# achinastone/Tensorium

Hardware: AMD Instinct MI355X
Metric: fp32 SGEMM GFLOP/s (M=N=K=4096) + YOLOv3 conv-fwd images/s (higher is better)
Workload: dtype fp32; 1 GPU; sgemm_nn_4096x4096x4096; M=4096, N=4096, K=4096, parallelism=1 independent replicas, one process per GPU, no data-path collective

## Files before the change

include/tns.h:

```cpp
#ifndef TNS_H
#define TNS_H

#include <stdint.h>
#include <stddef.h>

#ifdef __cplusplus
extern "C" {
#endif

#define TNS_ABI_VERSION 1

enum { TNS_CblasRowMajor = 101, TNS_CblasColMajor = 102 };
enum { TNS_CblasNoTrans = 111, TNS_CblasTrans = 112 };

enum {
  TNS_acLOGISTIC = 0, TNS_acRELU = 1, TNS_acRELU6 = 2, TNS_acRELIE = 3,
  TNS_acLINEAR = 4, TNS_acRAMP = 5, TNS_acTANH = 6, TNS_acPLSE = 7,
  TNS_acREVLEAKY = 8, TNS_acLEAKY = 9, TNS_acELU = 10, TNS_acLOGGY = 11,
  TNS_acSTAIR = 12, TNS_acHARDTAN = 13, TNS_acLHTAN = 14, TNS_acSELU = 15
};

enum {
  TNS_OK = 0,
  TNS_ERR_ARG = 1,
// ... 321 lines not shown
int         tns_conv_dw_tile_count(void);
int         tns_conv_tile_variant_count(void);
const char* tns_conv_tile_variant_name(int32_t variant);
int         tns_conv_slab_count(void);
const char* tns_conv_slab_name(int32_t variant);
int         tns_conv1x1_count(void);
const char* tns_conv1x1_name(int32_t variant);
int         tns_sdot_chains_variant_count(void);
const char* tns_sdot_chains_variant_name(int32_t variant);
int         tns_sdot_rc_variant_count(void);
const char* tns_sdot_rc_variant_name(int32_t variant);
const char* tns_gemm_variant_name(int32_t variant);
int tns_hip_gemm_variant(tns_ctx* ctx, int32_t variant, uint8_t transA, uint8_t transB,
                         int64_t M, int64_t N, int64_t K, float ALPHA,
                         const float* A, int64_t aOffset, int64_t lda, int64_t strideA,
                         const float* B, int64_t bOffset, int64_t ldb, int64_t strideB,
                         float BETA, float* C, int64_t cOffset, int64_t ldc, int64_t strideC,
                         int64_t batchCount);

enum { TNS_OPT_STRICT_BETA0 = 0, TNS_OPT_CONV_VARIANT = 1, TNS_OPT_CONV_PAD = 2,
       TNS_OPT_NT_SDOT = 3, TNS_OPT_SRSS_QUIRK = 4, TNS_OPT_TT_EXACT = 5,
       TNS_OPT_SDOT_FORM = 6, TNS_OPT_DX_FUSED = 7, TNS_OPT_DX_TILE = 8,
       TNS_OPT_DW_TILE = 9, TNS_OPT_BWD_OVERLAP = 10, TNS_OPT_DX_CONV = 11,
       TNS_OPT_DW_RES = 12, TNS_OPT_DERIVE_SUMS = 13, TNS_OPT_SCRATCH_CAP = 14 };
int tns_set_option(int32_t opt, int64_t value);

#ifdef __cplusplus
}
#endif
#endif
```

tensorium_amd/_abi.py:

```python
from __future__ import annotations

import ctypes as C
import os
import re
from pathlib import Path

PKG = Path(__file__).resolve().parent
ROOT = PKG.parent
LIB_PATH = PKG / "libtensorium_hip.so"
HEADER = ROOT / "include" / "tns.h"

i32, i64, u8, f32 = C.c_int32, C.c_int64, C.c_uint8, C.c_float
fptr = C.c_void_p
vp = C.c_void_p

CblasRowMajor, CblasColMajor = 101, 102
CblasNoTrans, CblasTrans = 111, 112
ACT = dict(LOGISTIC=0, RELU=1, RELU6=2, RELIE=3, LINEAR=4, RAMP=5, TANH=6, PLSE=7,
           REVLEAKY=8, LEAKY=9, ELU=10, LOGGY=11, STAIR=12, HARDTAN=13, LHTAN=14, SELU=15)
TNS_OK = 0
TNS_OP_GEMM, TNS_OP_IM2COL, TNS_OP_COL2IM, TNS_OP_BIAS, TNS_OP_ACTIVATE = range(5)
TNS_OPT_STRICT_BETA0 = 0
TNS_OPT_CONV_VARIANT, TNS_OPT_CONV_PAD, TNS_OPT_NT_SDOT, TNS_OPT_SRSS_QUIRK = 1, 2, 3, 4
TNS_OPT_TT_EXACT = 5
TNS_OPT_SDOT_FORM = 6
TNS_OPT_DX_FUSED = 7
TNS_OPT_DX_TILE = 8
TNS_OPT_DW_TILE = 9
TNS_OPT_BWD_OVERLAP = 10
TNS_OPT_DX_CONV = 11
TNS_OPT_DW_RES = 12
TNS_OPT_DERIVE_SUMS = 13
TNS_OPT_SCRATCH_CAP = 14

_CONV = [i64] * 11

PROTOTYPES: dict[str, tuple] = {
    "tns_abi_version": (C.c_int, []),
    "tns_last_error": (C.c_char_p, []),
    "tns_clear_error": (None, []),
    "tns_set_error_hook": (None, [vp]),
    "tns_device_count": (C.c_int, []),
    "tns_set_option": (C.c_int, [i32, i64]),
    "tns_cblas_sgemm": (None, [i32, i32, i32, i64, i64, i64, f32, fptr, i64, fptr, i64, f32,
                               fptr, i64]),
    "tns_cblas_sgemm_batch_strided": (None, [i32, i32, i32, i64, i64, i64, f32, fptr, i64, i64,
                                             fptr, i64, i64, f32, fptr, i64, i64, i64]),
    "tns_im2col": (None, [*_CONV, fptr, i64, fptr, i64, u8]),
    "tns_col2im": (None, [*_CONV, fptr, i64, fptr, i64, i64, u8]),
    "tns_im2col_strided_batched": (None, [*_CONV, fptr, i64, i64, fptr, i64, i64, i64]),
    "tns_col2im_strided_batched": (None, [*_CONV, fptr, i64, i64, fptr, i64, i64, i64]),
    "tns_hip_create": (C.c_int, [i32, C.POINTER(vp)]),
    "tns_hip_destroy": (C.c_int, [vp]),
    "tns_hip_set_stream": (C.c_int, [vp, vp]),
    "tns_hip_get_stream": (vp, [vp]),
    "tns_hip_pending_dw": (C.c_int, [vp]),
# ... 174 lines not shown
```

tensorium_amd/csrc/sgemm_nn_big.hip:

```cpp
#include <type_traits>

#include "tns_internal.hpp"

namespace tns {
namespace {

typedef float floatx16 __attribute__((ext_vector_type(16)));

template <int BM, int BN, int WM, int WN, int MINB, int BK = 32>
struct Geo {
  static constexpr int BM_ = BM, BN_ = BN, WN_ = WN, MINB_ = MINB, BK_ = BK;
  static constexpr int KQ = BK / 4;
  static constexpr int NT = 64 * WM * WN;
  static constexpr int WTM = BM / WM, WTN = BN / WN;
  static constexpr int TM = WTM / 32, TN = WTN / 32;
  static constexpr int LDA = BM, LDB = BN;
  static constexpr int A_TILE = BK * LDA, B_TILE = BK * LDB;
  static constexpr int STAGE = A_TILE + B_TILE;
  static constexpr int AU = BM * BK / 4 / NT;
  static constexpr int BROWS = 256 / BN;
  static constexpr int BDMA = BK / BROWS / (NT / 64);
  static_assert(TM == 2 || TM == 4, "A fragments read as one b64 / b128");
  static_assert(BN == 128 || BN == 256, "B rows of 512 B or 1 KB per DMA");
  static_assert(AU >= 1 && BDMA >= 1 && BM * BK / 4 % NT == 0, "staging split");
// ... 220 lines not shown
}

template <class G>
hipError_t launch(const GemmArgs& a, hipStream_t s) {
  if (!applies<G>(a)) return hipErrorInvalidValue;
  const int64_t tiles = (a.M / G::BM_) * (a.N / G::BN_);
  for (int64_t b0 = 0; b0 < a.batch; b0 += 65535) {
    GemmArgs sub = a;
    const int64_t nb = a.batch - b0 < 65535 ? a.batch - b0 : 65535;
    sub.A = a.A + b0 * a.strideA;
    sub.B = a.B + b0 * a.strideB;
    sub.C = a.C + b0 * a.strideC;
    sub.batch = nb;
    hipLaunchKernelGGL(sgemm_nn_big_kernel<G>, dim3((unsigned)tiles, (unsigned)nb), dim3(G::NT), 0,
                       s, sub);
    hipError_t e = hipGetLastError();
    if (e != hipSuccess) return e;
  }
  return hipSuccess;
}

}

int sgemm_nn_big_count() { return 9; }
const char* sgemm_nn_big_name(int v) {
  static const char* names[] = {"256x256x32_w2x4_nn_big", "128x128x32_w2x2_nn_big",
                                "256x128x32_w2x2_nn_big", "256x256x32_w4x4_nn_big",
                                "256x128x16_w2x2_b2_nn_big", "256x256x32_w2x4_pp_nn_big",
                                "256x256x32_w2x2_dma_nn_big", "256x256x32_w2x2_dma_flat_nn_big",
                                "256x256x32_w2x2_dma_b32_nn_big"};
  return v >= 0 && v < sgemm_nn_big_count() ? names[v] : "";
}

int sgemm_nn_big_pick(const GemmArgs& a) {
  if (applies<G256>(a) && (a.M / 256) * (a.N / 256) * a.batch >= 192)
    return sgemm_nn_w4_applies(a) ? 6 : sgemm_nn_pp_applies(a) ? 5 : 0;
  return -1;
}

hipError_t launch_sgemm_nn_big(int v, const GemmArgs& a, hipStream_t s) {
  switch (v) {
    case 0: return launch<G256>(a, s);
    case 1: return launch<G128>(a, s);
    case 2: return launch<G256x128>(a, s);
    case 3: return launch<G256w16>(a, s);
    case 4: return launch<G256x128k16>(a, s);
    case 5: return launch_sgemm_nn_pp(a, s);
    case 6: return launch_sgemm_nn_w4(a, s, true);
    case 7: return launch_sgemm_nn_w4(a, s, false);
    case 8: return launch_sgemm_nn_w4(a, s, true, false);
    default: return hipErrorInvalidValue;
  }
}

}
```

tensorium_amd/csrc/sgemm_nn_w4.hip:

```cpp
#include <type_traits>

#include "tns_internal.hpp"

namespace tns {
namespace {

typedef float floatx16 __attribute__((ext_vector_type(16)));
typedef float floatx4 __attribute__((ext_vector_type(4)));
typedef int int4v __attribute__((ext_vector_type(4)));
typedef const __attribute__((address_space(3))) float* lds_cptr;
typedef const __attribute__((address_space(3))) floatx4* lds_cptr4;

constexpr int BM = 256, BN = 256, BK = 32, NT = 256;
constexpr int A_TILE = BM * BK, B_TILE = BK * BN, STAGE = A_TILE + B_TILE;
constexpr int ROWS_MIN_TILES = 4;
constexpr int PRE_MIN_TILES = 8;

__device__ __forceinline__ void dma16(const float* sbase, unsigned voff, unsigned lds) {
  unsigned keep;
  asm volatile(
      "s_mov_b32 %0, m0\n\ts_mov_b32 m0, %3\n\ts_nop 0\n\t"
      "global_load_lds_dwordx4 %1, %2\n\ts_mov_b32 m0, %0"
      : "=&s"(keep)
      : "v"(voff), "s"(sbase), "s"(lds)
      : "memory");
}

#ifdef TNS_W4_STAMPS
#define TNS_W4_STAMP(i) stamp[i] = __builtin_amdgcn_s_memtime()
#else
#define TNS_W4_STAMP(i) \
  do {                  \
  } while (0)
#endif

template <bool ALPHA1, bool ROWS, bool PRE>
__global__ __launch_bounds__(NT, 1) void sgemm_nn_w4_kernel(GemmArgs p) {
  __shared__ __attribute__((aligned(16))) float smem[2 * STAGE];
#ifdef TNS_W4_STAMPS
  unsigned long long stamp[4];
  TNS_W4_STAMP(0);
#endif
  const int tid = threadIdx.x, lane = tid & 63;
  const int wid = __builtin_amdgcn_readfirstlane(tid >> 6);
  const int lc = lane & 31, h = lane >> 5;
  const int wm = wid >> 1, wn = wid & 1;

  const int tiles_m = (int)(p.M / BM), tiles_n = (int)(p.N / BN);
  int tm, tn;
  const int64_t bz = blockIdx.y;
  {
    const int nb = tiles_m * tiles_n, bid = blockIdx.x;
    const int xcd = bid & 7, q = nb >> 3, r = nb & 7;
    const int wg = (xcd < r ? xcd * (q + 1) : r * (q + 1) + (xcd - r) * q) + (bid >> 3);
    constexpr int GROUP_M = 8;
    const int per_group = GROUP_M * tiles_n;
    const int group = wg / per_group, first_m = group * GROUP_M;
    const int gsize = min(tiles_m - first_m, GROUP_M);
    const int in_group = wg - group * per_group;
    tm = first_m + in_group % gsize;
    tn = in_group / gsize;
  }
  const int64_t m0 = (int64_t)tm * BM, n0 = (int64_t)tn * BN;
  const float* __restrict__ A = p.A + bz * p.strideA;
  const float* __restrict__ B = p.B + bz * p.strideB;
  float* __restrict__ C = p.C + bz * p.strideC;
  const int64_t lda = p.lda, ldb = p.ldb, ldc = p.ldc;

  const int arow = lane >> 3;
  const unsigned a_voff = (unsigned)(arow * lda * 4) + 16u * (unsigned)((lane & 7) ^ ((arow >> 1) & 7));
  const unsigned a_voff1 = (unsigned)(arow * lda * 4) +
                           16u * (unsigned)((lane & 7) ^ (((arow >> 1) & 7) ^ 4));
  const unsigned b_voff0 = 16u * (unsigned)lane;
  const unsigned b_voff1 = 16u * (unsigned)((lane + 8) & 63);
  const unsigned lds0 = (unsigned)(uintptr_t)(__attribute__((address_space(3))) float*)smem;
  const float* a_row0 = A + m0 * lda;
  const float* b_row0 = B + n0;
  auto issue1 = [&](int u, int64_t k0, int st) {
    const unsigned sb = lds0 + (unsigned)(st * STAGE * 4);
    if (u < 8) {
      const int q = 8 * wid + u;
      dma16(a_row0 + (int64_t)(8 * q) * lda + k0, (u & 1) ? a_voff1 : a_voff,
            sb + (unsigned)(q * 1024));
    } else {
      const int r = 8 * wid + (u - 8);
      dma16(b_row0 + (k0 + r) * ldb, (u & 1) ? b_voff1 : b_voff0,
            sb + (unsigned)(A_TILE * 4 + r * 1024));
    }
  };
  auto issue = [&](int64_t k0, int st) {
    const unsigned sb = lds0 + (unsigned)(st * STAGE * 4);
#pragma unroll
    for (int u = 0; u < 8; ++u) {
      const int q = 8 * wid + u;
      dma16(a_row0 + (int64_t)(8 * q) * lda + k0, (u & 1) ? a_voff1 : a_voff,
            sb + (unsigned)(q * 1024));
    }
#pragma unroll
    for (int u = 0; u < 8; ++u) {
      const int r = 8 * wid + u;
      dma16(b_row0 + (k0 + r) * ldb, (u & 1) ? b_voff1 : b_voff0,
            sb + (unsigned)(A_TILE * 4 + r * 1024));
    }
  };

  const int nt = (int)(p.K / BK);

  floatx16 acc[4][4];
  const int64_t row_base = m0 + wm * 128;
  const __amdgpu_buffer_rsrc_t crs = __builtin_amdgcn_make_buffer_rsrc(
      C + row_base * ldc, 0, 0x7fffffff, 0x00020000);
  const unsigned c_voff = 4u * (unsigned)(4 * h * ldc + n0 + wn * 128 + 4 * lc);
  auto c_soff = [&](int i, int e) {
    return (unsigned)(4 * (32 * i + (e & 3) + 8 * (e >> 2)) * ldc);
  };

  const int swz = (lc >> 1) & 7;
  int b_col[4];
#pragma unroll
  for (int j = 0; j < 4; ++j)
    b_col[j] = A_TILE + h * BN + ((wn * 128 + 4 * lc + j - 32 * h) & 255);
  const float alpha = p.alpha;
  auto mma = [&](const float (&a)[4], const float (&b)[4]) {
    float aa[4];
#pragma unroll
    for (int i = 0; i < 4; ++i) aa[i] = ALPHA1 ? a[i] : alpha * a[i];
#pragma unroll
    for (int i = 0; i < 4; ++i)
#pragma unroll
      for (int j = 0; j < 4; ++j)
        acc[i][j] = __builtin_amdgcn_mfma_f32_32x32x2f32(aa[i], b[j], acc[i][j], 0, 0, 0);
  };
  auto mma_dma = [&](const float (&a)[4], const float (&b)[4], int64_t k0, int st, bool dma) {
    float aa[4];
#pragma unroll
    for (int i = 0; i < 4; ++i) aa[i] = ALPHA1 ? a[i] : alpha * a[i];
#pragma unroll
// ... 191 lines not shown
        after(s);
        rfrag(st, s + 2, I, fa0, fb0);
        __builtin_amdgcn_sched_barrier(0);
        rmma(I_, fa1, fb1);
        after(s + 1);
      }
      rfrag(st, BK / 2 - 1, I, fa1, fb1);
      __builtin_amdgcn_sched_barrier(0);
      rmma(I_, fa0, fb0);
      after(BK / 2 - 2);
      __builtin_amdgcn_sched_barrier(0);
      mid();
      if constexpr (NI >= 0) {
        rfrag(nst, 0, NI, fa0, fb0);
        __builtin_amdgcn_sched_barrier(0);
      }
      rmma(I_, fa1, fb1);
      after(BK / 2 - 1);
      __builtin_amdgcn_sched_barrier(0);
    };
    const float* const S0 = smem;
    const float* const S1 = smem + STAGE;

    int tb;
    if (p.beta_mode == BETA_ZERO) {
      issue(0, 0);
      issue(BK, 1);
#pragma unroll
      for (int i = 0; i < 4; ++i)
#pragma unroll
        for (int j = 0; j < 4; ++j) {
#pragma unroll
          for (int e = 0; e < 16; ++e) acc[i][j][e] = 0.0f;
          asm volatile("" : "+a"(acc[i][j]));
        }
      asm volatile("s_waitcnt vmcnt(16)" ::: "memory");
      bar();
      TNS_W4_STAMP(1);
      tb = 0;
    } else {
      const bool scale = p.beta_mode == BETA_SCALE;
      const float beta = p.beta;
      const uint64_t cb = (uint64_t)(uintptr_t)(C + row_base * ldc);
      const int4v crs_raw = {(int)(uint32_t)cb, (int)((uint32_t)(cb >> 32) & 0xffffu), 0x7fffffff,
                             0x00020000};
      floatx4 va[16], vb[16];
      auto ldrow = [&](int i, floatx4 (&v)[16]) {
#pragma unroll
        for (int e = 0; e < 16; ++e) {
          const unsigned so = c_soff(i, e);
          if (e == 0)
            asm volatile("s_nop 4\n\tbuffer_load_dwordx4 %0, %1, %2, %3 offen"
                         : "=&v"(v[e])
                         : "v"(c_voff), "s"(crs_raw), "s"(so)
                         : "memory");
          else
            asm volatile("buffer_load_dwordx4 %0, %1, %2, %3 offen"
                         : "=&v"(v[e])
                         : "v"(c_voff), "s"(crs_raw), "s"(so)
                         : "memory");
        }
      };
      auto waitrow = [&](auto N_, floatx4 (&v)[16]) {
        asm volatile("s_waitcnt vmcnt(%[n])"
                     : "+v"(v[0]), "+v"(v[1]), "+v"(v[2]), "+v"(v[3]), "+v"(v[4]), "+v"(v[5]),
                       "+v"(v[6]), "+v"(v[7])
                     : [n] "n"(decltype(N_)::value)
                     : "memory");
        asm volatile(""
                     : "+v"(v[8]), "+v"(v[9]), "+v"(v[10]), "+v"(v[11]), "+v"(v[12]), "+v"(v[13]),
                       "+v"(v[14]), "+v"(v[15])
                     :
                     : "memory");
      };
      auto mvrow = [&](auto I_, const floatx4 (&v)[16]) {
        constexpr int I = decltype(I_)::value;
#pragma unroll
        for (int j = 0; j < 4; ++j) {
#pragma unroll
          for (int e = 0; e < 16; ++e) {
            const float c = v[e][j];
            acc[I][j][e] = scale ? beta * c : c;
          }
          asm volatile("" : "+a"(acc[I][j]));
        }
      };
      using N0 = std::integral_constant<int, 0>;
      using N16 = std::integral_constant<int, 16>;
      using N32 = std::integral_constant<int, 32>;

      issue(0, 0);
      ldrow(0, va);
      issue(BK, 1);
      ldrow(1, vb);
      waitrow(N32{}, va);
      bar();
      mvrow(R0{}, va);
      ldrow(2, va);
      rfrag(S0, 0, 0, fa0, fb0);
      __builtin_amdgcn_sched_barrier(0);
      TNS_W4_STAMP(1);
      unit(R0{}, S0, R0{}, S1, [&] {
        asm volatile("s_waitcnt vmcnt(32)" ::: "memory");
        bar();
      }, none1);
      unit(R0{}, S1, R1{}, S0, [&] {
        waitrow(N16{}, vb);
        mvrow(R1{}, vb);
        ldrow(3, vb);
      }, none1);
      unit(R1{}, S0, R1{}, S1, none, none1);
      unit(R1{}, S1, R2{}, S0, [&] {
        waitrow(N16{}, va);
        mvrow(R2{}, va);
      }, none1);
      unit(R2{}, S0, R3{}, S0, [&] {
        waitrow(N0{}, vb);
        mvrow(R3{}, vb);
      }, none1);
      unit(R3{}, S0, R2{}, S1, none, none1);
      bar();
      unit(R2{}, S1, R3{}, S1, none, [&](int s) {
        if (s < 8) {
          issue1(2 * s, 2 * BK, 0);
          issue1(2 * s + 1, 2 * BK, 0);
        }
      });
      unit(R3{}, S1, RN{}, S1, none, none1);
      asm volatile("s_waitcnt vmcnt(0)" ::: "memory");
      bar();
      issue(3 * BK, 1);
      tb = 2;
    }

// ... 1 lines not shown
    const float* const sB = smem + ((nt + 1) & 1) * STAGE;
    if (tb < nt - 2) {
      if constexpr (PRE) {
        pre_init();
        pfrag(0, 0, a0, b0);
      } else {
        frag(S0, 0, a0, b0);
      }
      flat_loop(std::true_type{}, tb, nt - 2);
      fa0 = a0[0];
#pragma unroll
      for (int j = 0; j < 4; ++j) fb0[j] = b0[j];
    } else {
      rfrag(sA, 0, 0, fa0, fb0);
    }
    __builtin_amdgcn_sched_barrier(0);

    auto store1 = [&](auto I_, int e) {
      constexpr int I = decltype(I_)::value;
      const floatx4 v = {acc[I][0][e], acc[I][1][e], acc[I][2][e], acc[I][3][e]};
      __builtin_amdgcn_raw_buffer_store_b128(__builtin_bit_cast(int4v, v), crs, c_voff,
                                             c_soff(I, e), 0);
    };
    unit(R0{}, sA, R1{}, sA, none, none1);
    unit(R1{}, sA, R0{}, sB, [&] {
      asm volatile("s_waitcnt vmcnt(0)" ::: "memory");
      bar();
    }, none1);
    unit(R0{}, sB, R1{}, sB, none, none1);
    unit(R1{}, sB, R2{}, sA, none, [&](int s) { store1(R0{}, s); });
    unit(R2{}, sA, R2{}, sB, none, [&](int s) { store1(R1{}, s); });
    unit(R2{}, sB, R3{}, sA, none, none1);
    unit(R3{}, sA, R3{}, sB, none, [&](int s) { store1(R2{}, s); });
    unit(R3{}, sB, RN{}, sB, none, none1);
    TNS_W4_STAMP(2);
#pragma unroll
    for (int e = 0; e < 16; ++e) store1(R3{}, e);
  }
#ifdef TNS_W4_STAMPS
  asm volatile("s_waitcnt vmcnt(0)" ::: "memory");
  TNS_W4_STAMP(3);
  const unsigned blk = blockIdx.y * gridDim.x + blockIdx.x;
  if (lane == 0 && p.stamps != nullptr && blk < (1u << 16)) {
    unsigned long long* d = reinterpret_cast<unsigned long long*>(p.stamps) + (4 * blk + wid) * 4;
#pragma unroll
    for (int i = 0; i < 4; ++i) d[i] = stamp[i];
  }
#endif
}

bool aligned16(const void* q) { return (reinterpret_cast<uintptr_t>(q) & 15) == 0; }

#ifdef TNS_W4_STAMPS
unsigned* g_w4_stamps = nullptr;
#endif

}

bool sgemm_nn_w4_applies(const GemmArgs& a) {
  if (a.conv || a.epi != EPI_NONE || a.beta_mode == BETA_STORE) return false;
  if (a.M % BM || a.N % BN || a.K % BK || a.M <= 0 || a.N <= 0) return false;
  if (a.lda % 4 || a.ldb % 4 || !aligned16(a.A) || !aligned16(a.B)) return false;
  if (a.batch > 1 && (a.strideA % 4 || a.strideB % 4)) return false;
  if (a.lda * 4 * 8 > 0x7fffffffLL || (256 * a.ldc + a.N) * 4 > 0x7fffffffLL) return false;
  return (a.M / BM) * (a.N / BN) <= 0x7fffffff;
}

hipError_t launch_sgemm_nn_w4(const GemmArgs& a, hipStream_t s, bool rows, bool pre) {
  if (!sgemm_nn_w4_applies(a)) return hipErrorInvalidValue;
  const int64_t tiles = (a.M / BM) * (a.N / BN);
  const bool alpha1 = a.alpha == 1.0f;
  pre = pre && (!rows || a.K / BK >= PRE_MIN_TILES);
  rows = rows && a.K / BK >= ROWS_MIN_TILES;
  for (int64_t b0 = 0; b0 < a.batch; b0 += 65535) {
    GemmArgs sub = a;
    const int64_t nb = a.batch - b0 < 65535 ? a.batch - b0 : 65535;
    sub.A = a.A + b0 * a.strideA;
    sub.B = a.B + b0 * a.strideB;
    sub.C = a.C + b0 * a.strideC;
    sub.batch = nb;
#ifdef TNS_W4_STAMPS
    sub.stamps = g_w4_stamps;
#endif
    const dim3 grid((unsigned)tiles, (unsigned)nb);
    auto go = [&](auto R_, auto P_) {
      constexpr bool R = decltype(R_)::value, P = decltype(P_)::value;
      if (alpha1)
        hipLaunchKernelGGL((sgemm_nn_w4_kernel<true, R, P>), grid, dim3(NT), 0, s, sub);
      else
        hipLaunchKernelGGL((sgemm_nn_w4_kernel<false, R, P>), grid, dim3(NT), 0, s, sub);
    };
    if (rows && pre)
      go(std::true_type{}, std::true_type{});
    else if (rows)
      go(std::true_type{}, std::false_type{});
    else if (pre)
      go(std::false_type{}, std::true_type{});
    else
      go(std::false_type{}, std::false_type{});
    hipError_t e = hipGetLastError();
    if (e != hipSuccess) return e;
  }
  return hipSuccess;
}

#ifdef TNS_W4_STAMPS
extern "C" int tns_debug_w4_stamps(unsigned* dev_buf) {
  g_w4_stamps = dev_buf;
  return 0;
}
#endif

}
// ... 1 lines not shown
```

tensorium_amd/csrc/tns_api.cpp:

```cpp
#include <hip/hip_runtime.h>

#include <algorithm>
#include <cstdarg>
#include <cstdio>
#include <cstdlib>
#include <cstring>
#include <initializer_list>
#include <map>
#include <mutex>
#include <thread>
#include <vector>
#include <string>
#include <tuple>

#include "tns_ctx.hpp"

namespace tns {

static thread_local std::string g_err;
static tns_error_hook_t g_hook = nullptr;
static bool env_on(const char* name) { return !(getenv(name) && getenv(name)[0] == '0'); }
Options g_opt = [] {
  Options o;
  o.dx_c1 = env_on("TNS_DX_C1");
// ... 318 lines not shown
      g_opt.dx_fused = value < 0 ? 1 : (value > 2 ? 2 : value);
      return TNS_OK;
    case TNS_OPT_BWD_OVERLAP:
      g_opt.bwd_overlap = value <= 0 ? 0 : (value >= 2 ? 2 : 1);
      return TNS_OK;
    case TNS_OPT_DW_TILE:
      if (value >= dw_tile_count()) return set_error(TNS_ERR_ARG, "no dW tile %lld", (long long)value);
      g_opt.dw_tile = value < -1 ? -2 : value;
      return TNS_OK;
    case TNS_OPT_DX_TILE:
      if (value >= conv_tile4_ta_count()) return set_error(TNS_ERR_ARG, "no dX tile %lld", (long long)value);
      g_opt.dx_tile = value < -1 ? -2 : value;
      return TNS_OK;
    case TNS_OPT_DW_RES:
      if (value >= dw_res_count()) return set_error(TNS_ERR_ARG, "no dW res form %lld", (long long)value);
      g_opt.dw_res = value < -1 ? -2 : value;
      return TNS_OK;
    case TNS_OPT_DERIVE_SUMS:
      g_opt.derive_sums = value ? 1 : 0;
      return TNS_OK;
    case TNS_OPT_SCRATCH_CAP:
      g_opt.scratch_cap = value > 0 ? value : 0;
      return TNS_OK;
    case TNS_OPT_DX_CONV:
      if (value >= conv_tile4_dx3_count())
        return set_error(TNS_ERR_ARG, "no dX conv form %lld", (long long)value);
      g_opt.dx_conv = value < -1 ? -2 : value;
      return TNS_OK;
    default:
      return set_error(TNS_ERR_ARG, "unknown option %d", opt);
  }
}

int tns_hip_create(int32_t deviceIndex, tns_ctx** out) {
  if (!out) return set_error(TNS_ERR_ARG, "tns_hip_create: null out");
  *out = nullptr;
  int n = 0;
  hipError_t e = hipGetDeviceCount(&n);
  if (e != hipSuccess || n == 0)
    return set_error(TNS_ERR_HIP, "no HIP device available (%s)", hipGetErrorString(e));
  if (deviceIndex < 0 || deviceIndex >= n)
    return set_error(TNS_ERR_ARG, "device index %d out of range [0,%d)", deviceIndex, n);
  TNS_HIP_TRY(hipSetDevice(deviceIndex));
  tns_ctx* c = new tns_ctx();
  c->device = deviceIndex;
  {
// ... 1443 lines not shown
```

tensorium_amd/csrc/tns_ctx.hpp:

```cpp
#pragma once
#include <hip/hip_runtime.h>

#include <cstdlib>
#include <initializer_list>
#include <map>
#include <mutex>
#include <tuple>
#include <vector>

#include "tns_internal.hpp"

struct tns_ctx {
  int device = 0;
  hipStream_t stream = nullptr;
  bool own_stream = false;
  static constexpr int kSlots = 12;
  float* scratch[kSlots] = {};
  size_t scratch_elems[kSlots] = {};
  bool telemetry = false;
  double op_ms[TNS_OP_COUNT] = {0};
  hipEvent_t ev0 = nullptr, ev1 = nullptr;
  std::mutex mu;
  hipStream_t copy_stream = nullptr;
  std::vector<hipEvent_t> pipe_ev;
// ... 6 lines not shown
    uintptr_t lo[2], hi[2];
    uintptr_t wlo[2], whi[2];
  };
  std::vector<PendingDw> pending;
  uint32_t side_slots = 0;
  std::map<std::tuple<int64_t, int64_t, int64_t, int64_t, int64_t, int64_t, int64_t>, int*> ktabs;
};

namespace tns {

struct Options {
  int64_t strict_beta0 = 1;
  int64_t nt_sdot = 1;
  int64_t dx_fused = 1;
  int64_t dx_tile = -1;
  int64_t dx_conv = -1;
  int64_t dw_res = -1;
  bool dx_c1 = true;
  bool bn_fused = true;
  int64_t dw_tile = -1;
  int64_t bwd_overlap = 1;
  int64_t derive_sums = 0;
  int64_t scratch_cap = 0;
  int64_t tt_exact = 1;
  int64_t srss_quirk = 0;
  int64_t conv_variant = -1;
  int64_t conv_pad = -1;
};
extern Options g_opt;

enum { SLOT_COL = 0, SLOT_STAGE1 = 1, SLOT_STAGE2 = 2, SLOT_STAGE3 = 3, SLOT_DW = 4, SLOT_BN = 5,
       SLOT_MLP = 6, SLOT_WT = 7, SLOT_COL_DX = 8, SLOT_YOLO = 9, SLOT_RES_A = 10,
       SLOT_RES_B = 11, SLOT_COUNT = 12 };
static_assert(SLOT_COUNT == tns_ctx::kSlots, "one scratch buffer per slot");

inline int join_side(tns_ctx* c);

inline int ensure_scratch(tns_ctx* c, int slot, int64_t elems, float** out, bool side = false) {
  if (elems < 1) elems = 1;
  if (!side && c->side_pending && (c->side_slots >> slot & 1u) && c->stream != c->aux_stream)
    if (int r = join_side(c)) return r;
  if (g_opt.scratch_cap > 0 && elems > g_opt.scratch_cap)
    return set_error(TNS_ERR_NOMEM, "scratch slot %d: %lld floats exceed the cap of %lld", slot,
                     (long long)elems, (long long)g_opt.scratch_cap);
  if ((size_t)elems > c->scratch_elems[slot]) {
    if (c->scratch[slot]) {
// ... 221 lines not shown
```

tensorium_amd/csrc/tns_internal.hpp:

```cpp
#pragma once
#include <hip/hip_runtime.h>
#include <stdint.h>

#include "../../include/tns.h"

namespace tns {

int set_error(int code, const char* fmt, ...);
const char* hip_err_str(hipError_t e);

#define TNS_HIP_TRY(expr)                                                              \
  do {                                                                                 \
    hipError_t _e = (expr);                                                            \
    if (_e != hipSuccess)                                                              \
      return ::tns::set_error(TNS_ERR_HIP, "%s failed: %s (%s:%d)", #expr,            \
                              ::tns::hip_err_str(_e), __FILE__, __LINE__);             \
  } while (0)

enum EpiKind { EPI_NONE = 0, EPI_BIAS_ACT = 1, EPI_ADD = 2 };
constexpr bool act_transcendental(int act) { return act == 0 || act == 6; }

enum BetaMode { BETA_ZERO = 0, BETA_ONE = 1, BETA_SCALE = 2, BETA_STORE = 3 };

struct GemmArgs {
// ... 7 lines not shown
  float* C;
  int64_t ldc, strideC;
  int64_t batch;
  int epi;
  const float* bias;
  int act;
  int conv;
  const int* ktab;
  int ktab_n;
  int conv_H, conv_W, conv_ow, conv_ohw, conv_sY, conv_sX, conv_pH, conv_pW;
  int conv_bytes;
  int dx_cls, dx_taps, dx_imgW;
  unsigned* stamps;
};

hipError_t launch_sgemm(const GemmArgs& a, bool transA, bool transB, hipStream_t s);
int sgemm_nn_big_count();
const char* sgemm_nn_big_name(int v);
int sgemm_nn_big_pick(const GemmArgs& a);
hipError_t launch_sgemm_nn_big(int v, const GemmArgs& a, hipStream_t s);
bool sgemm_nn_pp_applies(const GemmArgs& a);
hipError_t launch_sgemm_nn_pp(const GemmArgs& a, hipStream_t s);
bool sgemm_nn_w4_applies(const GemmArgs& a);
hipError_t launch_sgemm_nn_w4(const GemmArgs& a, hipStream_t s, bool rows = true, bool pre = true);
hipError_t launch_sgemm_nt_sdot(const GemmArgs& a, hipStream_t s);
hipError_t launch_sdot_chains(const GemmArgs& a, int variant, hipStream_t s);
int sdot_chains_variant_count();
const char* sdot_chains_variant_name(int v);
int sdot_rc_variant_count();
const char* sdot_rc_variant_name(int v);
bool sdot_rc_applies(const GemmArgs& a);
hipError_t launch_sdot_rc(int v, const GemmArgs& a, hipStream_t s);
constexpr int SDOT_FORM_RC = 64;
void set_sdot_form(int form);
hipError_t launch_sgemm_tt(const GemmArgs& a, hipStream_t s);
hipError_t launch_add_in_order(float* C, const float* part, int64_t n, int64_t batch,
                               hipStream_t s);
hipError_t launch_sgemm_conv(const GemmArgs& a, hipStream_t s);
hipError_t launch_sgemm_conv_variant(int variant, const GemmArgs& a, hipStream_t s);
int conv_tile_count();
const char* conv_tile_name(int v);
int conv_tile_pick(const GemmArgs& a, int ks);
hipError_t launch_conv_tile(int v, const GemmArgs& a, int ks, int dil, hipStream_t s);
struct ConvSlabArgs {
  const float* input;
  const float* weights;
  const float* bias;
// ... 356 lines not shown
```

Before: 148,800 GFLOP/s.

## Add persistent-grid walk to w4 NN SGEMM with cross-tile prologue handover

Adds a persistent variant of the w4 DMA SGEMM kernel. A CU-sized grid walks successive output tiles, and the next tile's first K-stages and C rows are prefetched during the current tile's epilogue. The aim is to hide per-tile prologue and epilogue latency for small-K batched GEMMs, such as conv layers. The variant is selected only when K is between 128 and 1024 with enough work, so the 4096^3 SGEMM keeps the old path and only some YOLO conv GEMMs may change. The cost is extra complexity, s_nop padding in the DMA helper, and a changed unit schedule.

```diff
diff --git a/include/tns.h b/include/tns.h
--- a/include/tns.h
+++ b/include/tns.h
@@ -367,7 +367,8 @@
        TNS_OPT_NT_SDOT = 3, TNS_OPT_SRSS_QUIRK = 4, TNS_OPT_TT_EXACT = 5,
        TNS_OPT_SDOT_FORM = 6, TNS_OPT_DX_FUSED = 7, TNS_OPT_DX_TILE = 8,
        TNS_OPT_DW_TILE = 9, TNS_OPT_BWD_OVERLAP = 10, TNS_OPT_DX_CONV = 11,
-       TNS_OPT_DW_RES = 12, TNS_OPT_DERIVE_SUMS = 13, TNS_OPT_SCRATCH_CAP = 14 };
+       TNS_OPT_DW_RES = 12, TNS_OPT_DERIVE_SUMS = 13, TNS_OPT_SCRATCH_CAP = 14,
+       TNS_OPT_W4_PERS_GRID = 15 };
 int tns_set_option(int32_t opt, int64_t value);
 
 #ifdef __cplusplus
diff --git a/tensorium_amd/_abi.py b/tensorium_amd/_abi.py
--- a/tensorium_amd/_abi.py
+++ b/tensorium_amd/_abi.py
@@ -32,6 +32,7 @@
 TNS_OPT_DW_RES = 12
 TNS_OPT_DERIVE_SUMS = 13
 TNS_OPT_SCRATCH_CAP = 14
+TNS_OPT_W4_PERS_GRID = 15
 
 _CONV = [i64] * 11
 
diff --git a/tensorium_amd/csrc/sgemm_nn_big.hip b/tensorium_amd/csrc/sgemm_nn_big.hip
--- a/tensorium_amd/csrc/sgemm_nn_big.hip
+++ b/tensorium_amd/csrc/sgemm_nn_big.hip
@@ -1,5 +1,6 @@
 #include <type_traits>
 
+#include "tns_ctx.hpp"
 #include "tns_internal.hpp"
 
 namespace tns {
@@ -266,19 +267,30 @@
 
 }
 
-int sgemm_nn_big_count() { return 9; }
+int sgemm_nn_big_count() { return 10; }
 const char* sgemm_nn_big_name(int v) {
   static const char* names[] = {"256x256x32_w2x4_nn_big", "128x128x32_w2x2_nn_big",
                                 "256x128x32_w2x2_nn_big", "256x256x32_w4x4_nn_big",
                                 "256x128x16_w2x2_b2_nn_big", "256x256x32_w2x4_pp_nn_big",
                                 "256x256x32_w2x2_dma_nn_big", "256x256x32_w2x2_dma_flat_nn_big",
-                                "256x256x32_w2x2_dma_b32_nn_big"};
+                                "256x256x32_w2x2_dma_b32_nn_big",
+                                "256x256x32_w2x2_dma_pers_nn_big"};
   return v >= 0 && v < sgemm_nn_big_count() ? names[v] : "";
 }
 
+static int64_t w4_pers_grid() {
+  return g_opt.w4_pers_grid > 0 ? g_opt.w4_pers_grid : sgemm_nn_w4_cus();
+}
+
 int sgemm_nn_big_pick(const GemmArgs& a) {
-  if (applies<G256>(a) && (a.M / 256) * (a.N / 256) * a.batch >= 192)
-    return sgemm_nn_w4_applies(a) ? 6 : sgemm_nn_pp_applies(a) ? 5 : 0;
+  if (applies<G256>(a) && (a.M / 256) * (a.N / 256) * a.batch >= 192) {
+    if (!sgemm_nn_w4_applies(a)) return sgemm_nn_pp_applies(a) ? 5 : 0;
+    const int64_t g = w4_pers_grid();
+    const int64_t tiles = (a.M / 256) * (a.N / 256);
+    const bool walk = g > 0 && a.K >= 128 && a.K <= 1024 &&
+                      (a.batch >= 2 * g || tiles * a.batch >= 2 * g);
+    return walk ? 9 : 6;
+  }
   return -1;
 }
 
@@ -293,6 +305,10 @@
     case 6: return launch_sgemm_nn_w4(a, s, true);
     case 7: return launch_sgemm_nn_w4(a, s, false);
     case 8: return launch_sgemm_nn_w4(a, s, true, false);
+    case 9: {
+      const int64_t g = w4_pers_grid();
+      return g > 0 ? launch_sgemm_nn_w4(a, s, true, true, g) : hipErrorInvalidDevice;
+    }
     default: return hipErrorInvalidValue;
   }
 }
diff --git a/tensorium_amd/csrc/sgemm_nn_w4.hip b/tensorium_amd/csrc/sgemm_nn_w4.hip
--- a/tensorium_amd/csrc/sgemm_nn_w4.hip
+++ b/tensorium_amd/csrc/sgemm_nn_w4.hip
@@ -16,14 +16,23 @@
 constexpr int ROWS_MIN_TILES = 4;
 constexpr int PRE_MIN_TILES = 8;
 
+template <bool SPILLS = false>
 __device__ __forceinline__ void dma16(const float* sbase, unsigned voff, unsigned lds) {
   unsigned keep;
-  asm volatile(
-      "s_mov_b32 %0, m0\n\ts_mov_b32 m0, %3\n\ts_nop 0\n\t"
-      "global_load_lds_dwordx4 %1, %2\n\ts_mov_b32 m0, %0"
-      : "=&s"(keep)
-      : "v"(voff), "s"(sbase), "s"(lds)
-      : "memory");
+  if constexpr (SPILLS)
+    asm volatile(
+        "s_mov_b32 %0, m0\n\ts_mov_b32 m0, %3\n\ts_nop 2\n\t"
+        "global_load_lds_dwordx4 %1, %2\n\ts_mov_b32 m0, %0"
+        : "=&s"(keep)
+        : "v"(voff), "s"(sbase), "s"(lds)
+        : "memory");
+  else
+    asm volatile(
+        "s_mov_b32 %0, m0\n\ts_mov_b32 m0, %3\n\ts_nop 0\n\t"
+        "global_load_lds_dwordx4 %1, %2\n\ts_mov_b32 m0, %0"
+        : "=&s"(keep)
+        : "v"(voff), "s"(sbase), "s"(lds)
+        : "memory");
 }
 
 #ifdef TNS_W4_STAMPS
@@ -34,23 +43,26 @@
   } while (0)
 #endif
 
-template <bool ALPHA1, bool ROWS, bool PRE>
+template <bool ALPHA1, bool ROWS, bool PRE, bool PERS>
 __global__ __launch_bounds__(NT, 1) void sgemm_nn_w4_kernel(GemmArgs p) {
+  static_assert(ROWS || !PERS, "the persistent walk hands over between the rows schedule's ends");
   __shared__ __attribute__((aligned(16))) float smem[2 * STAGE];
-#ifdef TNS_W4_STAMPS
-  unsigned long long stamp[4];
-  TNS_W4_STAMP(0);
-#endif
   const int tid = threadIdx.x, lane = tid & 63;
   const int wid = __builtin_amdgcn_readfirstlane(tid >> 6);
   const int lc = lane & 31, h = lane >> 5;
   const int wm = wid >> 1, wn = wid & 1;
-
   const int tiles_m = (int)(p.M / BM), tiles_n = (int)(p.N / BN);
-  int tm, tn;
-  const int64_t bz = blockIdx.y;
-  {
-    const int nb = tiles_m * tiles_n, bid = blockIdx.x;
+  const int64_t lda = p.lda, ldb = p.ldb, ldc = p.ldc;
+
+  struct Tile {
+    const float* a_row0;
+    const float* b_row0;
+    float* c_rows;
+    unsigned c_voff;
+  };
+  auto tile_of = [&](const auto& g, int64_t bz, int bid) {
+    const int tiles_m = (int)(g.M / BM), tiles_n = (int)(g.N / BN);
+    const int nb = tiles_m * tiles_n;
     const int xcd = bid & 7, q = nb >> 3, r = nb & 7;
     const int wg = (xcd < r ? xcd * (q + 1) : r * (q + 1) + (xcd - r) * q) + (bid >> 3);
     constexpr int GROUP_M = 8;
@@ -58,14 +70,21 @@
     const int group = wg / per_group, first_m = group * GROUP_M;
     const int gsize = min(tiles_m - first_m, GROUP_M);
     const int in_group = wg - group * per_group;
-    tm = first_m + in_group % gsize;
-    tn = in_group / gsize;
-  }
-  const int64_t m0 = (int64_t)tm * BM, n0 = (int64_t)tn * BN;
-  const float* __restrict__ A = p.A + bz * p.strideA;
-  const float* __restrict__ B = p.B + bz * p.strideB;
-  float* __restrict__ C = p.C + bz * p.strideC;
-  const int64_t lda = p.lda, ldb = p.ldb, ldc = p.ldc;
+    const int tm = first_m + in_group % gsize;
+    const int tn = in_group / gsize;
+    const int64_t m0 = (int64_t)tm * BM, n0 = (int64_t)tn * BN;
+    Tile t;
+    t.a_row0 = g.A + bz * g.strideA + m0 * g.lda;
+    t.b_row0 = g.B + bz * g.strideB + n0;
+    t.c_rows = g.C + bz * g.strideC + (m0 + wm * 128) * g.ldc;
+    t.c_voff = 4u * (unsigned)(4 * h * g.ldc + n0 + wn * 128 + 4 * lc);
+    return t;
+  };
+  int64_t item_bz = PERS ? (int64_t)(blockIdx.x / (unsigned)(tiles_m * tiles_n)) : (int64_t)blockIdx.y;
+  int item_bid = PERS ? (int)(blockIdx.x % (unsigned)(tiles_m * tiles_n)) : (int)blockIdx.x;
+  Tile cur = tile_of(p, item_bz, item_bid);
+  bool handed = false;
+  floatx4 va[16], vb[16];
 
   const int arow = lane >> 3;
   const unsigned a_voff = (unsigned)(arow * lda * 4) + 16u * (unsigned)((lane & 7) ^ ((arow >> 1) & 7));
@@ -74,45 +93,73 @@
   const unsigned b_voff0 = 16u * (unsigned)lane;
   const unsigned b_voff1 = 16u * (unsigned)((lane + 8) & 63);
   const unsigned lds0 = (unsigned)(uintptr_t)(__attribute__((address_space(3))) float*)smem;
-  const float* a_row0 = A + m0 * lda;
-  const float* b_row0 = B + n0;
-  auto issue1 = [&](int u, int64_t k0, int st) {
+  const int nt = (int)(p.K / BK);
+
+#ifdef TNS_W4_STAMPS
+  unsigned long long held[4] = {};
+  int64_t held_item = -1;
+  auto put_stamps = [&](int64_t it, const unsigned long long (&st)[4]) {
+    if (lane == 0 && p.stamps != nullptr && it >= 0 && it < (1 << 16)) {
+      unsigned long long* d = reinterpret_cast<unsigned long long*>(p.stamps) + (4 * it + wid) * 4;
+#pragma unroll
+      for (int i = 0; i < 4; ++i) d[i] = st[i];
+    }
+  };
+#endif
+  for (;;) {
+#ifdef TNS_W4_STAMPS
+  unsigned long long stamp[4];
+  TNS_W4_STAMP(0);
+  const int64_t stamp_item = PERS ? item_bz * (tiles_m * tiles_n) + item_bid
+                                  : (int64_t)blockIdx.y * gridDim.x + blockIdx.x;
+#endif
+  Tile nxt = cur;
+  bool more = false;
+  const float* const a_row0 = cur.a_row0;
+  const float* const b_row0 = cur.b_row0;
+
+  auto issue1_at = [&](const float* ar, const float* br, int u, int64_t k0, int st) {
     const unsigned sb = lds0 + (unsigned)(st * STAGE * 4);
     if (u < 8) {
       const int q = 8 * wid + u;
-      dma16(a_row0 + (int64_t)(8 * q) * lda + k0, (u & 1) ? a_voff1 : a_voff,
+      dma16<PERS>(ar + (int64_t)(8 * q) * lda + k0, (u & 1) ? a_voff1 : a_voff,
             sb + (unsigned)(q * 1024));
     } else {
       const int r = 8 * wid + (u - 8);
-      dma16(b_row0 + (k0 + r) * ldb, (u & 1) ? b_voff1 : b_voff0,
+      dma16<PERS>(br + (k0 + r) * ldb, (u & 1) ? b_voff1 : b_voff0,
             sb + (unsigned)(A_TILE * 4 + r * 1024));
     }
   };
-  auto issue = [&](int64_t k0, int st) {
+  auto issue1 = [&](int u, int64_t k0, int st) { issue1_at(a_row0, b_row0, u, k0, st); };
+  auto issue_at = [&](const float* ar, const float* br, int64_t k0, int st) {
     const unsigned sb = lds0 + (unsigned)(st * STAGE * 4);
 #pragma unroll
     for (int u = 0; u < 8; ++u) {
       const int q = 8 * wid + u;
-      dma16(a_row0 + (int64_t)(8 * q) * lda + k0, (u & 1) ? a_voff1 : a_voff,
+      dma16<PERS>(ar + (int64_t)(8 * q) * lda + k0, (u & 1) ? a_voff1 : a_voff,
             sb + (unsigned)(q * 1024));
     }
 #pragma unroll
     for (int u = 0; u < 8; ++u) {
       const int r = 8 * wid + u;
-      dma16(b_row0 + (k0 + r) * ldb, (u & 1) ? b_voff1 : b_voff0,
+      dma16<PERS>(br + (k0 + r) * ldb, (u & 1) ? b_voff1 : b_voff0,
             sb + (unsigned)(A_TILE * 4 + r * 1024));
     }
   };
-
-  const int nt = (int)(p.K / BK);
+  auto issue = [&](int64_t k0, int st) { issue_at(a_row0, b_row0, k0, st); };
 
   floatx16 acc[4][4];
-  const int64_t row_base = m0 + wm * 128;
   const __amdgpu_buffer_rsrc_t crs = __builtin_amdgcn_make_buffer_rsrc(
-      C + row_base * ldc, 0, 0x7fffffff, 0x00020000);
-  const unsigned c_voff = 4u * (unsigned)(4 * h * ldc + n0 + wn * 128 + 4 * lc);
+      cur.c_rows, 0, 0x7fffffff, 0x00020000);
+  const unsigned c_voff = cur.c_voff;
   auto c_soff = [&](int i, int e) {
-    return (unsigned)(4 * (32 * i + (e & 3) + 8 * (e >> 2)) * ldc);
+    if constexpr (PERS) {
+      unsigned l = (unsigned)ldc;
+      asm volatile("" : "+s"(l));
+      return (unsigned)(4 * (32 * i + (e & 3) + 8 * (e >> 2))) * l;
+    } else {
+      return (unsigned)(4 * (32 * i + (e & 3) + 8 * (e >> 2)) * ldc);
+    }
   };
 
   const int swz = (lc >> 1) & 7;
@@ -350,10 +397,65 @@
     const float* const S0 = smem;
     const float* const S1 = smem + STAGE;
 
+    const bool scale = p.beta_mode == BETA_SCALE;
+    const float beta = p.beta;
+    auto raw_rsrc = [](const float* rows) {
+      const uint64_t cb = (uint64_t)(uintptr_t)rows;
+      const int4v r = {(int)(uint32_t)cb, (int)((uint32_t)(cb >> 32) & 0xffffu), 0x7fffffff,
+                       0x00020000};
+      return r;
+    };
+    auto ldrow_at = [&](const int4v crs_t, unsigned voff, int i, floatx4 (&v)[16]) {
+#pragma unroll
+      for (int e = 0; e < 16; ++e) {
+        const unsigned so = c_soff(i, e);
+        if (PERS || e == 0)
+          asm volatile("s_nop 4\n\tbuffer_load_dwordx4 %0, %1, %2, %3 offen"
+                       : "=&v"(v[e])
+                       : "v"(voff), "s"(crs_t), "s"(so)
+                       : "memory");
+        else
+          asm volatile("buffer_load_dwordx4 %0, %1, %2, %3 offen"
+                       : "=&v"(v[e])
+                       : "v"(voff), "s"(crs_t), "s"(so)
+                       : "memory");
+      }
+    };
+    auto waitrow = [&](auto N_, floatx4 (&v)[16]) {
+      asm volatile("s_waitcnt vmcnt(%[n])"
+                   : "+v"(v[0]), "+v"(v[1]), "+v"(v[2]), "+v"(v[3]), "+v"(v[4]), "+v"(v[5]),
+                     "+v"(v[6]), "+v"(v[7])
+                   : [n] "n"(decltype(N_)::value)
+                   : "memory");
+      asm volatile(""
+                   : "+v"(v[8]), "+v"(v[9]), "+v"(v[10]), "+v"(v[11]), "+v"(v[12]), "+v"(v[13]),
+                     "+v"(v[14]), "+v"(v[15])
+                   :
+                   : "memory");
+    };
+    auto mvrow = [&](auto I_, const floatx4 (&v)[16]) {
+      constexpr int I = decltype(I_)::value;
+#pragma unroll
+      for (int j = 0; j < 4; ++j) {
+#pragma unroll
+        for (int e = 0; e < 16; ++e) {
+          const float c = v[e][j];
+          acc[I][j][e] = scale ? beta * c : c;
+        }
+        asm volatile("" : "+a"(acc[I][j]));
+      }
+    };
+    using N0 = std::integral_constant<int, 0>;
+    using N16 = std::integral_constant<int, 16>;
+    using N32 = std::integral_constant<int, 32>;
+    using N48 = std::integral_constant<int, 48>;
+
     int tb;
     if (p.beta_mode == BETA_ZERO) {
-      issue(0, 0);
-      issue(BK, 1);
+      if (!(PERS && handed)) {
+        issue(0, 0);
+        issue(BK, 1);
+      }
 #pragma unroll
       for (int i = 0; i < 4; ++i)
 #pragma unroll
@@ -362,82 +464,51 @@
           for (int e = 0; e < 16; ++e) acc[i][j][e] = 0.0f;
           asm volatile("" : "+a"(acc[i][j]));
         }
-      asm volatile("s_waitcnt vmcnt(16)" ::: "memory");
-      bar();
+      if (!(PERS && handed)) {
+        asm volatile("s_waitcnt vmcnt(16)" ::: "memory");
+        bar();
+      }
       TNS_W4_STAMP(1);
       tb = 0;
     } else {
-      const bool scale = p.beta_mode == BETA_SCALE;
-      const float beta = p.beta;
-      const uint64_t cb = (uint64_t)(uintptr_t)(C + row_base * ldc);
-      const int4v crs_raw = {(int)(uint32_t)cb, (int)((uint32_t)(cb >> 32) & 0xffffu), 0x7fffffff,
-                             0x00020000};
-      floatx4 va[16], vb[16];
-      auto ldrow = [&](int i, floatx4 (&v)[16]) {
-#pragma unroll
-        for (int e = 0; e < 16; ++e) {
-          const unsigned so = c_soff(i, e);
-          if (e == 0)
-            asm volatile("s_nop 4\n\tbuffer_load_dwordx4 %0, %1, %2, %3 offen"
-                         : "=&v"(v[e])
-                         : "v"(c_voff), "s"(crs_raw), "s"(so)
-                         : "memory");
-          else
-            asm volatile("buffer_load_dwordx4 %0, %1, %2, %3 offen"
-                         : "=&v"(v[e])
-                         : "v"(c_voff), "s"(crs_raw), "s"(so)
-                         : "memory");
-        }
-      };
-      auto waitrow = [&](auto N_, floatx4 (&v)[16]) {
-        asm volatile("s_waitcnt vmcnt(%[n])"
-                     : "+v"(v[0]), "+v"(v[1]), "+v"(v[2]), "+v"(v[3]), "+v"(v[4]), "+v"(v[5]),
-                       "+v"(v[6]), "+v"(v[7])
-                     : [n] "n"(decltype(N_)::value)
-                     : "memory");
-        asm volatile(""
-                     : "+v"(v[8]), "+v"(v[9]), "+v"(v[10]), "+v"(v[11]), "+v"(v[12]), "+v"(v[13]),
-                       "+v"(v[14]), "+v"(v[15])
-                     :
-                     : "memory");
-      };
-      auto mvrow = [&](auto I_, const floatx4 (&v)[16]) {
-        constexpr int I = decltype(I_)::value;
-#pragma unroll
-        for (int j = 0; j < 4; ++j) {
-#pragma unroll
-          for (int e = 0; e < 16; ++e) {
-            const float c = v[e][j];
-            acc[I][j][e] = scale ? beta * c : c;
-          }
-          asm volatile("" : "+a"(acc[I][j]));
-        }
-      };
-      using N0 = std::integral_constant<int, 0>;
-      using N16 = std::integral_constant<int, 16>;
-      using N32 = std::integral_constant<int, 32>;
-
-      issue(0, 0);
-      ldrow(0, va);
-      issue(BK, 1);
-      ldrow(1, vb);
-      waitrow(N32{}, va);
-      bar();
+      const int4v crs_raw = raw_rsrc(cur.c_rows);
+      auto ldrow = [&](int i, floatx4 (&v)[16]) { ldrow_at(crs_raw, c_voff, i, v); };
+      if (!(PERS && handed)) {
+        issue(0, 0);
+        ldrow(0, va);
+        issue(BK, 1);
+        ldrow(1, vb);
+        waitrow(N32{}, va);
+        bar();
+      }
       mvrow(R0{}, va);
       ldrow(2, va);
       rfrag(S0, 0, 0, fa0, fb0);
       __builtin_amdgcn_sched_barrier(0);
       TNS_W4_STAMP(1);
-      unit(R0{}, S0, R0{}, S1, [&] {
-        asm volatile("s_waitcnt vmcnt(32)" ::: "memory");
-        bar();
-      }, none1);
-      unit(R0{}, S1, R1{}, S0, [&] {
-        waitrow(N16{}, vb);
-        mvrow(R1{}, vb);
-        ldrow(3, vb);
-      }, none1);
-      unit(R1{}, S0, R1{}, S1, none, none1);
+      if constexpr (!PERS) {
+        unit(R0{}, S0, R0{}, S1, [&] {
+          asm volatile("s_waitcnt vmcnt(32)" ::: "memory");
+          bar();
+        }, none1);
+        unit(R0{}, S1, R1{}, S0, [&] {
+          waitrow(N16{}, vb);
+          mvrow(R1{}, vb);
+          ldrow(3, vb);
+        }, none1);
+        unit(R1{}, S0, R1{}, S1, none, none1);
+      } else {
+        unit(R0{}, S0, R1{}, S0, [&] {
+          if (!handed) waitrow(N16{}, vb);
+          mvrow(R1{}, vb);
+          ldrow(3, vb);
+        }, none1);
+        unit(R1{}, S0, R0{}, S1, [&] {
+          asm volatile("s_waitcnt vmcnt(48)" ::: "memory");
+          bar();
+        }, none1);
+        unit(R0{}, S1, R1{}, S1, none, none1);
+      }
       unit(R1{}, S1, R2{}, S0, [&] {
         waitrow(N16{}, va);
         mvrow(R2{}, va);
@@ -485,31 +556,107 @@
       __builtin_amdgcn_raw_buffer_store_b128(__builtin_bit_cast(int4v, v), crs, c_voff,
                                              c_soff(I, e), 0);
     };
-    unit(R0{}, sA, R1{}, sA, none, none1);
-    unit(R1{}, sA, R0{}, sB, [&] {
-      asm volatile("s_waitcnt vmcnt(0)" ::: "memory");
-      bar();
-    }, none1);
-    unit(R0{}, sB, R1{}, sB, none, none1);
-    unit(R1{}, sB, R2{}, sA, none, [&](int s) { store1(R0{}, s); });
-    unit(R2{}, sA, R2{}, sB, none, [&](int s) { store1(R1{}, s); });
-    unit(R2{}, sB, R3{}, sA, none, none1);
-    unit(R3{}, sA, R3{}, sB, none, [&](int s) { store1(R2{}, s); });
-    unit(R3{}, sB, RN{}, sB, none, none1);
-    TNS_W4_STAMP(2);
-#pragma unroll
-    for (int e = 0; e < 16; ++e) store1(R3{}, e);
+    if constexpr (!PERS) {
+      unit(R0{}, sA, R1{}, sA, none, none1);
+      unit(R1{}, sA, R0{}, sB, [&] {
+        asm volatile("s_waitcnt vmcnt(0)" ::: "memory");
+        bar();
+      }, none1);
+      unit(R0{}, sB, R1{}, sB, none, none1);
+      unit(R1{}, sB, R2{}, sA, none, [&](int s) { store1(R0{}, s); });
+      unit(R2{}, sA, R2{}, sB, none, [&](int s) { store1(R1{}, s); });
+      unit(R2{}, sB, R3{}, sA, none, none1);
+      unit(R3{}, sA, R3{}, sB, none, [&](int s) { store1(R2{}, s); });
+      unit(R3{}, sB, RN{}, sB, none, none1);
+      TNS_W4_STAMP(2);
+#pragma unroll
+      for (int e = 0; e < 16; ++e) store1(R3{}, e);
+    } else {
+      {
+        typedef const __attribute__((address_space(4))) GemmArgs* kernarg_ptr;
+        kernarg_ptr g = (kernarg_ptr)__builtin_amdgcn_kernarg_segment_ptr();
+        asm volatile("" : "+s"(g));
+        const int nb = (int)(g->M / BM) * (int)(g->N / BN);
+        int bid = item_bid + (int)(gridDim.x % (unsigned)nb);
+        int64_t bz = item_bz + (int64_t)(gridDim.x / (unsigned)nb);
+        if (bid >= nb) {
+          bid -= nb;
+          ++bz;
+        }
+        more = bz < g->batch;
+        item_bid = bid;
+        item_bz = bz;
+        if (more) nxt = tile_of(*g, bz, bid);
+      }
+      const bool hand = more && !(nt & 1);
+      const bool loadc = p.beta_mode != BETA_ZERO;
+      const int4v crs_nxt = raw_rsrc(nxt.c_rows);
+#ifdef TNS_W4_STAMPS
+      put_stamps(held_item, held);
+      held_item = -1;
+#endif
+      unit(R0{}, sA, R1{}, sA, none, none1);
+      unit(R1{}, sA, R2{}, sA, none, none1);
+      unit(R2{}, sA, R3{}, sA, none, none1);
+      unit(R3{}, sA, R0{}, sB, [&] {
+        asm volatile("s_waitcnt vmcnt(0)" ::: "memory");
+        bar();
+      }, none1);
+#pragma unroll
+      for (int e = 0; e < 16; ++e) asm volatile("" : "=v"(va[e]), "=v"(vb[e]));
+      if (hand && loadc) {
+        ldrow_at(crs_nxt, nxt.c_voff, 0, va);
+        ldrow_at(crs_nxt, nxt.c_voff, 1, vb);
+      }
+      unit(R0{}, sB, R1{}, sB, none, [&](int s) {
+        if (hand && s < 8) {
+          issue1_at(nxt.a_row0, nxt.b_row0, 2 * s, 0, 0);
+          issue1_at(nxt.a_row0, nxt.b_row0, 2 * s + 1, 0, 0);
+        }
+      });
+      unit(R1{}, sB, R2{}, sB, none, [&](int s) { store1(R0{}, s); });
+      unit(R2{}, sB, R3{}, sB, none, [&](int s) { store1(R1{}, s); });
+      unit(R3{}, sB, RN{}, sB, none, [&](int s) { store1(R2{}, s); });
+      TNS_W4_STAMP(2);
+      if (hand) {
+        if (loadc) {
+          waitrow(N48{}, va);
+          asm volatile(""
+                       : "+v"(vb[0]), "+v"(vb[1]), "+v"(vb[2]), "+v"(vb[3]), "+v"(vb[4]),
+                         "+v"(vb[5]), "+v"(vb[6]), "+v"(vb[7])
+                       :
+                       : "memory");
+          asm volatile(""
+                       : "+v"(vb[8]), "+v"(vb[9]), "+v"(vb[10]), "+v"(vb[11]), "+v"(vb[12]),
+                         "+v"(vb[13]), "+v"(vb[14]), "+v"(vb[15])
+                       :
+                       : "memory");
+        } else {
+          asm volatile("s_waitcnt vmcnt(48)" ::: "memory");
+        }
+        bar();
+        issue_at(nxt.a_row0, nxt.b_row0, BK, 1);
+      }
+#pragma unroll
+      for (int e = 0; e < 16; ++e) store1(R3{}, e);
+      if (more && !hand) bar();
+      handed = hand;
+    }
   }
 #ifdef TNS_W4_STAMPS
-  asm volatile("s_waitcnt vmcnt(0)" ::: "memory");
+  if (!(PERS && more)) asm volatile("s_waitcnt vmcnt(0)" ::: "memory");
   TNS_W4_STAMP(3);
-  const unsigned blk = blockIdx.y * gridDim.x + blockIdx.x;
-  if (lane == 0 && p.stamps != nullptr && blk < (1u << 16)) {
-    unsigned long long* d = reinterpret_cast<unsigned long long*>(p.stamps) + (4 * blk + wid) * 4;
-#pragma unroll
-    for (int i = 0; i < 4; ++i) d[i] = stamp[i];
+  if (PERS && more) {
+#pragma unroll
+    for (int i = 0; i < 4; ++i) held[i] = stamp[i];
+    held_item = stamp_item;
+  } else {
+    put_stamps(stamp_item, stamp);
   }
 #endif
+  if (!PERS || !more) break;
+  cur = nxt;
+  }
 }
 
 bool aligned16(const void* q) { return (reinterpret_cast<uintptr_t>(q) & 15) == 0; }
@@ -529,12 +676,45 @@
   return (a.M / BM) * (a.N / BN) <= 0x7fffffff;
 }
 
-hipError_t launch_sgemm_nn_w4(const GemmArgs& a, hipStream_t s, bool rows, bool pre) {
+int sgemm_nn_w4_cus() {
+  constexpr int kMaxDev = 64;
+  static int cus[kMaxDev] = {};
+  int dev = 0;
+  if (hipGetDevice(&dev) != hipSuccess || dev < 0 || dev >= kMaxDev) return 0;
+  if (cus[dev] == 0) {
+    int n = 0;
+    if (hipDeviceGetAttribute(&n, hipDeviceAttributeMultiprocessorCount, dev) != hipSuccess)
+      return 0;
+    cus[dev] = n;
+  }
+  return cus[dev];
+}
+
+hipError_t launch_sgemm_nn_w4(const GemmArgs& a, hipStream_t s, bool rows, bool pre,
+                              int64_t pers_grid) {
   if (!sgemm_nn_w4_applies(a)) return hipErrorInvalidValue;
   const int64_t tiles = (a.M / BM) * (a.N / BN);
   const bool alpha1 = a.alpha == 1.0f;
   pre = pre && (!rows || a.K / BK >= PRE_MIN_TILES);
   rows = rows && a.K / BK >= ROWS_MIN_TILES;
+  if (pers_grid > 0 && rows) {
+    GemmArgs sub = a;
+#ifdef TNS_W4_STAMPS
+    sub.stamps = g_w4_stamps;
+#endif
+    int64_t blocks = pers_grid < 0x7fffffffLL ? pers_grid : 0x7fffffffLL;
+    if (a.batch < blocks && tiles * a.batch < blocks) blocks = tiles * a.batch;
+    const dim3 grid((unsigned)blocks);
+    if (alpha1 && pre)
+      hipLaunchKernelGGL((sgemm_nn_w4_kernel<true, true, true, true>), grid, dim3(NT), 0, s, sub);
+    else if (alpha1)
+      hipLaunchKernelGGL((sgemm_nn_w4_kernel<true, true, false, true>), grid, dim3(NT), 0, s, sub);
+    else if (pre)
+      hipLaunchKernelGGL((sgemm_nn_w4_kernel<false, true, true, true>), grid, dim3(NT), 0, s, sub);
+    else
+      hipLaunchKernelGGL((sgemm_nn_w4_kernel<false, true, false, true>), grid, dim3(NT), 0, s, sub);
+    return hipGetLastError();
+  }
   for (int64_t b0 = 0; b0 < a.batch; b0 += 65535) {
     GemmArgs sub = a;
     const int64_t nb = a.batch - b0 < 65535 ? a.batch - b0 : 65535;
@@ -549,9 +729,9 @@
     auto go = [&](auto R_, auto P_) {
       constexpr bool R = decltype(R_)::value, P = decltype(P_)::value;
       if (alpha1)
-        hipLaunchKernelGGL((sgemm_nn_w4_kernel<true, R, P>), grid, dim3(NT), 0, s, sub);
+        hipLaunchKernelGGL((sgemm_nn_w4_kernel<true, R, P, false>), grid, dim3(NT), 0, s, sub);
       else
-        hipLaunchKernelGGL((sgemm_nn_w4_kernel<false, R, P>), grid, dim3(NT), 0, s, sub);
+        hipLaunchKernelGGL((sgemm_nn_w4_kernel<false, R, P, false>), grid, dim3(NT), 0, s, sub);
     };
     if (rows && pre)
       go(std::true_type{}, std::true_type{});
diff --git a/tensorium_amd/csrc/tns_api.cpp b/tensorium_amd/csrc/tns_api.cpp
--- a/tensorium_amd/csrc/tns_api.cpp
+++ b/tensorium_amd/csrc/tns_api.cpp
@@ -364,6 +364,9 @@
     case TNS_OPT_SCRATCH_CAP:
       g_opt.scratch_cap = value > 0 ? value : 0;
       return TNS_OK;
+    case TNS_OPT_W4_PERS_GRID:
+      g_opt.w4_pers_grid = value > 0 ? (value < 0x7fffffffLL ? value : 0x7fffffffLL) : 0;
+      return TNS_OK;
     case TNS_OPT_DX_CONV:
       if (value >= conv_tile4_dx3_count())
         return set_error(TNS_ERR_ARG, "no dX conv form %lld", (long long)value);
diff --git a/tensorium_amd/csrc/tns_ctx.hpp b/tensorium_amd/csrc/tns_ctx.hpp
--- a/tensorium_amd/csrc/tns_ctx.hpp
+++ b/tensorium_amd/csrc/tns_ctx.hpp
@@ -52,6 +52,7 @@
   int64_t bwd_overlap = 1;
   int64_t derive_sums = 0;
   int64_t scratch_cap = 0;
+  int64_t w4_pers_grid = 0;
   int64_t tt_exact = 1;
   int64_t srss_quirk = 0;
   int64_t conv_variant = -1;
diff --git a/tensorium_amd/csrc/tns_internal.hpp b/tensorium_amd/csrc/tns_internal.hpp
--- a/tensorium_amd/csrc/tns_internal.hpp
+++ b/tensorium_amd/csrc/tns_internal.hpp
@@ -53,7 +53,9 @@
 bool sgemm_nn_pp_applies(const GemmArgs& a);
 hipError_t launch_sgemm_nn_pp(const GemmArgs& a, hipStream_t s);
 bool sgemm_nn_w4_applies(const GemmArgs& a);
-hipError_t launch_sgemm_nn_w4(const GemmArgs& a, hipStream_t s, bool rows = true, bool pre = true);
+hipError_t launch_sgemm_nn_w4(const GemmArgs& a, hipStream_t s, bool rows = true, bool pre = true,
+                              int64_t pers_grid = 0);
+int sgemm_nn_w4_cus();
 hipError_t launch_sgemm_nt_sdot(const GemmArgs& a, hipStream_t s);
 hipError_t launch_sdot_chains(const GemmArgs& a, int variant, hipStream_t s);
 int sdot_chains_variant_count();
```

Result: no change. 148,700 GFLOP/s (-0.1%).
